# dan-lee-gh/monte-carlo-gp

Hardware: AMD Instinct MI355X
Metric: race-simulations/sec (20 drivers, 60 laps) (higher is better)
Workload: dtype f64

## Files before the change

### monte_carlo_gp_amd/csrc/mcgp_hip.hip

```cpp
#include "../../include/mcgp.h"
#include "params_build.h"
#include "race_kernel.hip.h"
#include "race_kernel_reg.hip.h"
#include "championship.hip.h"
#include "champ_rounds.hip.h"
#include "matchups.hip.h"
#include "resume.hip.h"
#include "trace.hip.h"
#include "strategy.hip.h"
#include "gaps.hip.h"
#include "conditions.hip.h"
#include "stints.hip.h"
#include "moves.hip.h"
#include "fastest.hip.h"
#include "champ_bonus.hip.h"
#include "plan_pack.h"
#include "champ_pack.h"

#define MCGP_FE_FN __host__ __device__ static inline
#include "frontend_exp.h"
#include "elo_update.h"
#include "normal53_table.h"

#include <hip/hip_runtime.h>
// ... 193 lines not shown
    c.d_fe_in = c.d_fe_out = c.d_norm53 = nullptr;
    c.d_fe_pen = nullptr;
    c.work.release();
    if (c.call_start) (void)hipEventDestroy(c.call_start);
    if (c.call_stop) (void)hipEventDestroy(c.call_stop);
    c.call_start = c.call_stop = nullptr;
    for (auto &t : c.timer) {
        if (t.start) (void)hipEventDestroy(t.start);
        if (t.stop) (void)hipEventDestroy(t.stop);
        if (t.d_ticket) (void)hipFree(t.d_ticket);
        t.retire.release();
        t = DeviceCtx::Timer{};
    }
    c.last_timer = -1;
}

size_t lds_limit(size_t device_bytes)
{
    if (const char *e = std::getenv("MCGP_LDS_PER_BLOCK")) {
        const unsigned long long v = std::strtoull(e, nullptr, 10);
        if (v >= 16384 && v < device_bytes) return (size_t)v;
    }
    return device_bytes;
}

int init_ctx_body(int device, DeviceCtx &c)
{
    HIP_TRY(hipSetDevice(device));
    hipDeviceProp_t prop;
    HIP_TRY(hipGetDeviceProperties(&prop, device));
    c.cu_count = prop.multiProcessorCount;
    c.lds_per_block = lds_limit(prop.sharedMemPerBlock);
    for (auto &sl : c.slot) {
        HIP_TRY(hipMalloc(&sl.dev, sizeof(mcgp::KParams)));
        HIP_TRY(hipHostMalloc(&sl.host, sizeof(mcgp::KParams)));
        HIP_TRY(hipEventCreateWithFlags(&sl.uploaded, hipEventDisableTiming));
    }
    HIP_TRY(hipMalloc(&c.d_hist, sizeof(unsigned long long) * MCGP_MAX_CARS * MCGP_MAX_CARS));
    HIP_TRY(hipMalloc(&c.d_grid, MCGP_MAX_CARS));
    HIP_TRY(hipMalloc(&c.d_order1, MCGP_MAX_CARS));
    HIP_TRY(hipMalloc(&c.d_fe_in, sizeof(double) * 4 * MCGP_MAX_CARS));
    HIP_TRY(hipMalloc(&c.d_fe_pen, sizeof(int32_t) * MCGP_MAX_CARS));
    HIP_TRY(hipMalloc(&c.d_fe_out, sizeof(double) * MCGP_MAX_CARS * MCGP_MAX_CARS));
    HIP_TRY(hipMalloc(&c.d_norm53, sizeof(mcgp_normal53_table_bits)));
    HIP_TRY(hipMemcpy(c.d_norm53, mcgp_normal53_table_bits, sizeof(mcgp_normal53_table_bits), hipMemcpyHostToDevice));
    HIP_TRY(hipFuncSetAttribute(reinterpret_cast<const void *>(&mcgp::race_kernel),
                                hipFuncAttributeMaxDynamicSharedMemorySize, (int)c.lds_per_block));
    HIP_TRY(hipFuncSetAttribute(reinterpret_cast<const void *>(&mcgp::race_resume_kernel),
                                hipFuncAttributeMaxDynamicSharedMemorySize, (int)c.lds_per_block));
    HIP_TRY(hipFuncSetAttribute(reinterpret_cast<const void *>(&mcgp::race_trace_kernel),
                                hipFuncAttributeMaxDynamicSharedMemorySize, (int)c.lds_per_block));
    return MCGP_OK;
}

int ensure_ctx_locked(int device, DeviceCtx &c)
{
    if (c.ready) return MCGP_OK;
    const int rc = init_ctx_body(device, c);
    if (rc != MCGP_OK) {
        release_ctx(c);
        return rc;
    }
    c.ready = true;
    return MCGP_OK;
}

int build_params(const mcgp_config *cfg, const mcgp_drivers *drv, const double *grid_probs, uint32_t n,
                 mcgp::KParams *kp)
{
    const char *err = "";
    const int rc = mcgp::build_params(cfg, drv, grid_probs, n, kp, &err);
    return rc == MCGP_OK ? rc : fail(rc, err);
}

using KernelFn = void (*)(const mcgp::KParams *, uint64_t, uint64_t, uint32_t, uint32_t, unsigned long long *,
                          uint8_t *, const uint8_t *, uint32_t, uint32_t *, uint32_t *);

}

namespace mcgp {
#define X(N_)                                                                                                                   \
    extern template __global__ void race_kernel_reg<N_>(const KParams *, uint64_t, uint64_t, uint32_t, uint32_t,               \
                                                        unsigned long long *, uint8_t *, const uint8_t *, uint32_t, uint32_t *, \
                                                        uint32_t *);                                                           \
    extern template __global__ void race_kernel_reg<N_, kSmallBlockWaves>(const KParams *, uint64_t, uint64_t, uint32_t,       \
                                                                          uint32_t, unsigned long long *, uint8_t *,           \
                                                                          const uint8_t *, uint32_t, uint32_t *, uint32_t *);  \
    extern template __global__ void race_kernel_reg_wide<N_>(const KParams *, uint64_t, uint64_t, uint32_t, uint32_t,          \
                                                             unsigned long long *, uint8_t *, const uint8_t *, uint32_t,       \
                                                             uint32_t *, uint32_t *, const double *);                          \
    extern template __global__ void race_kernel_reg_batch<N_>(const KParams *, const BatchItem *, uint32_t, uint64_t,          \
                                                              unsigned long long *, uint32_t, uint32_t *, uint32_t *);
MCGP_REG_SIZES(X)
#undef X
}

namespace {

using BatchKernelFn = void (*)(const mcgp::KParams *, const mcgp::BatchItem *, uint32_t, uint64_t, unsigned long long *,
                               uint32_t, uint32_t *, uint32_t *);
using WideKernelFn = void (*)(const mcgp::KParams *, uint64_t, uint64_t, uint32_t, uint32_t, unsigned long long *,
                              uint8_t *, const uint8_t *, uint32_t, uint32_t *, uint32_t *, const double *);

struct RegKernels {
    KernelFn reg, small;
    WideKernelFn wide;
    BatchKernelFn batch;
};
const RegKernels kRegKernels[] = {
#define X(N_) {&mcgp::race_kernel_reg<N_>, &mcgp::race_kernel_reg<N_, mcgp::kSmallBlockWaves>, \
               &mcgp::race_kernel_reg_wide<N_>, &mcgp::race_kernel_reg_batch<N_>},
    MCGP_REG_SIZES(X)
#undef X
};
static_assert(sizeof(kRegKernels) / sizeof(kRegKernels[0]) == MCGP_MAX_CARS, "one entry per field size 1..32");

const RegKernels *reg_kernels(uint32_t n) { return n >= 1 && n <= MCGP_MAX_CARS ? &kRegKernels[n - 1] : nullptr; }

bool force_generic()
{
    const char *e = std::getenv("MCGP_FORCE_GENERIC");
    return e && e[0] == '1';
}

KernelFn select_kernel(const mcgp::KParams &kp, bool *is_reg)
{
    const RegKernels *rk = reg_kernels((uint32_t)kp.n);
    *is_reg = rk && !force_generic() && mcgp::reg_kernel_serves(kp);
    return *is_reg ? rk->reg : &mcgp::race_kernel;
}

int check_wide(const mcgp::KParams &kp)
{
// ... 173 lines not shown
int launch(DeviceCtx &c, const mcgp::KParams &kp, uint64_t n_sims, uint64_t sim_offset, uint64_t seed,
           hipStream_t stream, unsigned long long *d_hist, uint8_t *d_orders, const uint8_t *d_fixed_grid,
           const FrontEnd &fe = FrontEnd())
{
    if (n_sims == 0) return MCGP_OK;
    bool is_reg = false;
    KernelFn kernel = select_kernel(kp, &is_reg);
    WideKernelFn wide = nullptr;
    if (kp.wide) {
        const int rc = check_wide(kp);
        if (rc != MCGP_OK) return rc;
        wide = reg_kernels((uint32_t)kp.n)->wide;
        HIP_TRY(hipFuncSetAttribute(reinterpret_cast<const void *>(wide), hipFuncAttributeMaxDynamicSharedMemorySize,
                                    (int)c.lds_per_block));
        is_reg = true;
        kernel = nullptr;
    }
    DeviceCtx::Slot *sl = nullptr;
    if (!fe.on)
        for (auto &cand : c.slot)
            if (cand.used && cand.shareable && std::memcmp(cand.host, &kp, sizeof(kp)) == 0) { sl = &cand; break; }
    if (!sl) {
        sl = &c.slot[c.next_slot];
        c.next_slot = (c.next_slot + 1) % kParamSlots;
        if (sl->used)
            for (auto &rd : sl->reader)
                if (rd.live) {
                    HIP_TRY(hipEventSynchronize(rd.done));
                    rd.live = false;
                }
        std::memcpy(sl->host, &kp, sizeof(kp));
        sl->used = true;
        sl->shareable = !fe.on;
        HIP_TRY(hipMemcpyAsync(sl->dev, sl->host, sizeof(kp), hipMemcpyHostToDevice, stream));
        if (fe.on) {
            hipLaunchKernelGGL(grid_probs_kernel, dim3(1), dim3(mcgp::kMaxCars), 0, stream, c.d_fe_in, c.d_fe_pen,
                               (int)kp.n, sl->dev->grid_probs);
            HIP_TRY(hipGetLastError());
        }
        HIP_TRY(hipEventRecord(sl->uploaded, stream));
        sl->upload_stream = stream;
    } else if (sl->upload_stream != stream) {
        HIP_TRY(hipStreamWaitEvent(stream, sl->uploaded, 0));
    }
    int ti = -1;
    {
        const int rc = claim_timer(c, stream, &ti);
        if (rc != MCGP_OK) return rc;
    }
    c.timer[ti].seq = ++c.timer_seq;
    if (!c.timer[ti].d_ticket) return fail(MCGP_E_HIP, "no work counter for this stream");
    HIP_TRY(hipEventRecord(c.timer[ti].start, stream));
    const uint64_t cap = max_sims_per_launch();
    uint32_t grid = 0, block = 0, lds = 0;
    bool small_shape = false;
    auto resource_error = [](hipError_t e) {
        return e == hipErrorOutOfMemory || e == hipErrorInvalidValue || e == hipErrorLaunchOutOfResources ||
               e == hipErrorInvalidConfiguration;
    };
    for (uint64_t done = 0; done < n_sims; done += cap) {
        const uint64_t m = (n_sims - done) < cap ? (n_sims - done) : cap;
        for (;;) {
            const KernelFn k = small_shape ? reg_kernels((uint32_t)kp.n)->small : kernel;
            launch_geometry(c, (uint32_t)kp.n, is_reg, wide ? reinterpret_cast<KernelFn>(wide) : k, m, &grid, &block, &lds,
                            wide ? mcgp::wide_block_waves(kp.n) : small_shape ? mcgp::kSmallBlockWaves : 0, wide != nullptr,
                            kp.total_laps);
            const bool may_shrink = is_reg && !wide && !small_shape;
// ... 356 lines not shown
int32_t mcgp_run_batch(uint32_t n_problems, const mcgp_config *cfgs, const mcgp_drivers *drvs,
                       const double *const *grid_probs, uint32_t n, uint64_t n_sims, const uint64_t *sim_offsets,
                       const uint64_t *seeds, int32_t device, uint64_t *hist_out)
{
    if (!cfgs || !drvs || !grid_probs || !seeds || !hist_out) return fail(MCGP_E_BAD_ARG, "a batch array is NULL");
    if (n_problems < 1 || n_problems > 4096) return fail(MCGP_E_BAD_ARG, "n_problems must be in [1, 4096]");
    if (n_sims >= 0xFFFFFE00ull) return fail(MCGP_E_BAD_ARG, "n_sims per problem must be below 2^32 - 512 in a batch");
    if (n_sims == 0) return MCGP_OK;
    std::vector<mcgp::KParams> kps;
    std::vector<mcgp::BatchItem> items;
    std::vector<uint32_t> shared_index, solo_index;
    std::vector<mcgp::KParams> solo_kps;
    const bool generic = force_generic();
    const RegKernels *rk = reg_kernels(n);
    {
        mcgp::KParams kp;
        for (uint32_t p = 0; p < n_problems; ++p) {
            if (!grid_probs[p]) return fail(MCGP_E_BAD_ARG, "a grid_probs pointer of the batch is NULL");
            int rc = build_params(&cfgs[p], &drvs[p], grid_probs[p], n, &kp);
            if (rc == MCGP_OK) rc = check_wide(kp);
            if (rc != MCGP_OK) return rc;
            if (!rk || generic || kp.wide || !mcgp::reg_kernel_serves(kp)) {
                solo_index.push_back(p);
                solo_kps.push_back(kp);
            } else {
                shared_index.push_back(p);
                kps.push_back(kp);
                items.push_back(mcgp::BatchItem{sim_offsets ? sim_offsets[p] : 0ull, seeds[p]});
            }
        }
    }
    const uint32_t n_shared = (uint32_t)kps.size();
    const size_t cells = (size_t)n * n;
    Counts counts;
    const int rc = on_device(device, true, [&](DeviceCtx &c) -> int {
        const int waves = mcgp::reg_block_waves((int)n);
        const uint32_t block = (uint32_t)waves * 64u;
        const size_t lds = mcgp::shared_lds_bytes_reg((int)n) + (size_t)block * mcgp::per_thread_lds_bytes_reg((int)n) +
                           mcgp::kBatchLdsExtra;
        int reg_cap = 4 * mcgp::reg_min_waves((int)n);
        int blocks_per_cu = (int)(c.lds_per_block / lds);
        if (blocks_per_cu * waves > reg_cap) blocks_per_cu = reg_cap / waves;
        if (blocks_per_cu < 1) blocks_per_cu = 1;
        const uint32_t n_chunks = (uint32_t)((n_sims + 63) / 64);
        const uint64_t n_tasks = ((uint64_t)n_shared * n_chunks + (uint64_t)waves - 1) / (uint64_t)waves;
        uint64_t grid = (uint64_t)c.cu_count * (uint64_t)blocks_per_cu;
        if (grid > n_tasks) grid = n_tasks;
        Layout ws;
        const size_t o_kps = ws.add(sizeof(mcgp::KParams) * n_shared), o_items = ws.add(sizeof(mcgp::BatchItem) * n_shared);
        const size_t o_hist = ws.add(sizeof(unsigned long long) * cells * n_problems);
        const size_t o_ticket = ws.add(sizeof(uint32_t) * n_shared);
        const size_t o_retire = ws.add(mcgp::reg_retire_ws_bytes((int)n, (size_t)grid * block));
        int r = c.work.reserve(ws.bytes);
        if (r != MCGP_OK) return r;
        unsigned long long *d_hist = c.work.at<unsigned long long>(o_hist);
        HIP_TRY(hipMemsetAsync(d_hist, 0, o_retire - o_hist, nullptr));
        if (n_shared) {
            const BatchKernelFn kernel = rk->batch;
            HIP_TRY(hipFuncSetAttribute(reinterpret_cast<const void *>(kernel), hipFuncAttributeMaxDynamicSharedMemorySize,
                                        (int)c.lds_per_block));
            HIP_TRY(hipMemcpyAsync(c.work.at(o_kps), kps.data(), sizeof(mcgp::KParams) * n_shared, hipMemcpyHostToDevice, nullptr));
            HIP_TRY(hipMemcpyAsync(c.work.at(o_items), items.data(), sizeof(mcgp::BatchItem) * n_shared, hipMemcpyHostToDevice,
                                   nullptr));
            hipLaunchKernelGGL(kernel, dim3((uint32_t)grid), dim3(block), lds, nullptr, c.work.at<const mcgp::KParams>(o_kps),
                               c.work.at<const mcgp::BatchItem>(o_items), n_shared, n_sims, d_hist, n_chunks,
                               c.work.at<uint32_t>(o_ticket), c.work.at<uint32_t>(o_retire));
            HIP_TRY(hipGetLastError());
            note_launch(c, (uint32_t)grid, block, (uint32_t)lds, "mcgp::race_kernel_reg_batch<%u>", n);
        }
        for (size_t j = 0; j < solo_index.size(); ++j) {
            const uint32_t p = solo_index[j];
            r = launch(c, solo_kps[j], n_sims, sim_offsets ? sim_offsets[p] : 0ull, seeds[p], nullptr,
                       d_hist + (n_shared + j) * cells, nullptr, nullptr);
            if (r != MCGP_OK) return r;
        }
        return counts.download(d_hist, cells * n_problems);
    });
    if (rc != MCGP_OK) return rc;
    std::vector<Counts::Seg> segs;
    for (uint32_t p : shared_index) segs.push_back({hist_out + (size_t)p * cells, cells});
    for (uint32_t p : solo_index) segs.push_back({hist_out + (size_t)p * cells, cells});
    counts.add_to(segs);
    return MCGP_OK;
}

struct ChampRoundsOut {
    uint64_t *round_hist, *contend, *secure, *team_round_hist, *team_contend, *team_secure;
};

struct ChampBonus {
    const int32_t *points, *within;
    uint64_t *bonus_hist, *fastest_hist;
};

static int32_t run_championship(uint32_t n_races, const mcgp_config *cfgs, const mcgp_drivers *drvs,
                                const double *const *grid_probs, uint32_t n, uint64_t n_sims, uint64_t sim_offset,
                                const uint64_t *seeds, const int32_t *points, const uint8_t *countback,
                                const int32_t *init_points, const int32_t *init_counts, const int32_t *team,
                                uint32_t n_teams, int32_t device, uint64_t *champ_hist, uint64_t *team_hist,
// ... 1047 lines not shown
```

### monte_carlo_gp_amd/csrc/params_build.h

```cpp
#pragma once
#include "../../include/mcgp.h"
#include "normal_table.h"
#include "race_common.hip.h"

#include <cmath>
#include <cstring>

namespace mcgp {

inline uint64_t threshold(double p)
{
    if (!(p > 0.0)) return 0;
    const double x = p * 4294967296.0;
    if (x >= 4294967296.0) return 4294967296ull;
    return (uint64_t)std::ceil(x);
}

inline uint64_t threshold53(double p)
{
    if (!(p > 0.0)) return 0;
    const double x = p * 9007199254740992.0;
    if (x >= 9007199254740992.0) return 9007199254740992ull;
    return (uint64_t)std::ceil(x);
}
// ... 48 lines not shown
        if (cfg->comp_optimal_laps[c] < 0 || cfg->comp_optimal_laps[c] > 50000)
            { *err = "comp_optimal_laps out of range"; return MCGP_E_BAD_ARG; }
    }
    for (uint32_t d = 0; d < n; ++d) {
        const double deg = drv->tire_deg[d];
        kp->base_pace[d] = drv->base_pace[d];
        kp->factor[d] = deg > 0 ? deg / 0.05 : 1.0;
        kp->tire_deg[d] = deg;
        kp->variance[d] = drv->variance[d];
        kp->t_dnf1[d] = threshold(drv->team_dnf[d] * 4.0);
        kp->t_dnf[d] = threshold(drv->lap_dnf[d]);
        kp->t53_dnf1[d] = threshold53(drv->team_dnf[d] * 4.0);
        kp->q64_dnf[d] = survival64(drv->lap_dnf[d]);
        const double pit_deg = drv->tire_deg_pit[d];
        for (int c = 0; c < 5; ++c) {
            int opt = cfg->comp_optimal_laps[c];
            if (pit_deg > 0.05) opt = (int)((double)opt * 0.85);
            else if (pit_deg < 0.02) opt = (int)((double)opt * 1.1);
            kp->opt_laps[d * kCompStride + c] = (uint16_t)opt;
        }
    }
    if (grid_probs)
        for (uint32_t d = 0; d < n; ++d)
            for (uint32_t s = 0; s < n; ++s) {
                const double p = grid_probs[(size_t)d * n + s];
                if (!(p >= 0.0)) { *err = "grid_probs has a negative or NaN entry"; return MCGP_E_BAD_ARG; }
                kp->grid_probs[(size_t)d * n + s] = p;
            }
    static_assert(sizeof(mcgp_normal_table_bits) == sizeof(kp->normal_bits), "normal table size");
    std::memcpy(kp->normal_bits, mcgp_normal_table_bits, sizeof(kp->normal_bits));
    return MCGP_OK;
}

}
```

### monte_carlo_gp_amd/csrc/race_common.hip.h

```cpp
#pragma once
#include <hip/hip_runtime.h>
#include <stdint.h>

namespace mcgp {

constexpr int kMaxCars = 32;
constexpr int kNormalRows = 448;
constexpr int kNormal53Rows = 784;
constexpr int kNormal53RowBytes = 64;
constexpr int kCompStride = 8;

constexpr uint32_t kPurposeGrid = 0u << 16;
constexpr uint32_t kPurposeEvent = 1u << 16;
constexpr uint32_t kPurposeCar = 2u << 16;
constexpr uint32_t kPurposeOvt = 3u << 16;
constexpr uint32_t kPurposeRetire = 4u << 16;

__host__ __device__ inline uint32_t retire_next_threshold(uint32_t S, uint32_t q)
{
    return (uint32_t)(((uint64_t)S * (uint64_t)q) >> 32);
}
__host__ __device__ inline uint32_t draw_retirement_lap(uint32_t w, uint64_t t, int L)
{
    if (t == 0ull) return 0u;
    const uint32_t q = (uint32_t)(4294967296ull - t);
    uint32_t S = q;
    for (int k = 2; k <= L; ++k) {
        if (!(w < S)) return (uint32_t)k;
        S = retire_next_threshold(S, q);
    }
    return 0u;
}
__host__ __device__ inline uint32_t draw_retirement_lap_after(uint32_t w, uint64_t t, int k, int L)
{
    const uint32_t r = draw_retirement_lap(w, t, L - k + 1);
    return r == 0u ? 0u : (uint32_t)(k - 1) + r;
}

struct KParams {
    int32_t n, total_laps, track, pop_sh, pop_mh, pad0;
    double pit_loss, overtake_delta, drs_delta, dirty_thr, dirty_pen;
    double overtake_delta_31;
    uint64_t t_red, t_sc, t_vsc, t_vsc_tire;
    double comp_deg[kCompStride], comp_delta[kCompStride];
    double base_pace[kMaxCars];
    double factor[kMaxCars];
    double tire_deg[kMaxCars];
    double variance[kMaxCars];
    uint64_t t_dnf1[kMaxCars];
    uint64_t t_dnf[kMaxCars];
    uint16_t opt_laps[kMaxCars * kCompStride];
    double grid_probs[kMaxCars * kMaxCars];
    uint32_t normal_bits[kNormalRows * 4];
    int32_t wide, pad1;
    uint64_t t53_red, t53_sc, t53_vsc, t53_vsc_tire;
    uint64_t t53_dnf1[kMaxCars];
    uint64_t q64_dnf[kMaxCars];
};

constexpr size_t kSharedTableBytes =
    kNormalRows * 16
    + 4 * kMaxCars * 8
    + 2 * kMaxCars * 8
    + kMaxCars * kCompStride * 2
    + 2 * kCompStride * 8
    + kMaxCars * kMaxCars * 4;
__host__ __device__ constexpr size_t per_thread_lds_bytes(int n) { return (size_t)n * (8 + 8 + 4 + 1 + 2); }

__device__ __forceinline__ uint32_t xor3_key(uint32_t a, uint32_t b, uint32_t key)
{
#if defined(__HIP_DEVICE_COMPILE__)
    uint32_t r;
    asm("v_bitop3_b32 %0, %1, %2, %3 bitop3:0x96" : "=v"(r) : "v"(a), "v"(b), "s"(key));
    return r;
#else
    return a ^ b ^ key;
#endif
}

__device__ __forceinline__ void philox4x32_10(uint32_t c0, uint32_t c1, uint32_t c2, uint32_t c3,
                                              uint32_t k0, uint32_t k1,
                                              uint32_t &o0, uint32_t &o1, uint32_t &o2, uint32_t &o3)
{
#pragma unroll
    for (int r = 0; r < 10; ++r) {
        const uint64_t p0 = (uint64_t)0xD2511F53u * c0;
        const uint64_t p1 = (uint64_t)0xCD9E8D57u * c2;
        const uint32_t n0 = xor3_key((uint32_t)(p1 >> 32), c1, k0);
        const uint32_t n2 = xor3_key((uint32_t)(p0 >> 32), c3, k1);
        c1 = (uint32_t)p1;
        c3 = (uint32_t)p0;
// ... 93 lines not shown
```

### monte_carlo_gp_amd/csrc/race_isa.hip.h

```cpp
#ifndef MCGP_RACE_ISA_H
#define MCGP_RACE_ISA_H
#include <hip/hip_runtime.h>

namespace mcgp {

__device__ __forceinline__ void minmax_f64(double a, double b, double &lo, double &hi)
{
    asm("v_min_f64 %0, %1, %2" : "=v"(lo) : "v"(a), "v"(b));
    asm("v_max_f64 %0, %1, %2" : "=v"(hi) : "v"(a), "v"(b));
}

__device__ __forceinline__ double max_f64(double a, double b)
{
    double r;
    asm("v_max_f64 %0, %1, %2" : "=v"(r) : "v"(a), "v"(b));
    return r;
}

__device__ __forceinline__ double max_abs_f64(double a, double b)
{
    double r;
    asm("v_max_f64 %0, |%1|, %2" : "=v"(r) : "v"(a), "v"(b));
    return r;
}
// ... 384 lines not shown
{
    const int lo = __builtin_amdgcn_readlane(__double2loint(x), lane);
    const int hi = __builtin_amdgcn_readlane(__double2hiint(x), lane);
    return __hiloint2double(hi, lo);
}
__device__ __forceinline__ double bpermute_f64(double x, int src_lane)
{
    const int lo = __builtin_amdgcn_ds_bpermute(src_lane << 2, __double2loint(x));
    const int hi = __builtin_amdgcn_ds_bpermute(src_lane << 2, __double2hiint(x));
    return __hiloint2double(hi, lo);
}
__device__ __forceinline__ uint32_t next_ticket(uint32_t *counter, uint32_t , uint32_t , int )
{
    uint32_t t = 0u;
    if (__builtin_amdgcn_mbcnt_hi(~0u, __builtin_amdgcn_mbcnt_lo(~0u, 0u)) == 0u)
        t = __hip_atomic_fetch_add(counter, 1u, __ATOMIC_RELAXED, __HIP_MEMORY_SCOPE_AGENT);
    return (uint32_t)__builtin_amdgcn_readfirstlane((int)t);
}
__device__ __forceinline__ uint32_t peek_ticket(const uint32_t *counter)
{
    return __hip_atomic_load(counter, __ATOMIC_RELAXED, __HIP_MEMORY_SCOPE_AGENT);
}
__device__ __forceinline__ uint32_t first_lane_with(bool pred)
{
    const unsigned long long m = __ballot(pred);
    return m ? (uint32_t)__builtin_ctzll(m) : 64u;
}
#define MCGP_ANY(pred) (__any((int)(pred)) != 0)
__device__ __forceinline__ void pin(uint32_t &x) { asm volatile("" : "+v"(x)); }
__device__ __forceinline__ void pin(double &x) { asm volatile("" : "+v"(x)); }
__device__ __forceinline__ void pin_scalar(uint32_t &x) { asm volatile("" : "+s"(x)); }
template <typename T>
__device__ __forceinline__ void pin_ptr(const T *&p) { asm volatile("" : "+s"(p)); }

__device__ __forceinline__ uint32_t lds_base_of(const void *p)
{
    return (uint32_t)(uintptr_t)(const MCGP_LDS void *)p;
}

}
#endif
```

### monte_carlo_gp_amd/csrc/race_kernel_reg.hip.h

```cpp
#pragma once
#include "race_common.hip.h"
#include "race_isa.hip.h"
#include "sort_networks.h"

#include <utility>

#ifndef MCGP_STAT
#define MCGP_STAT(what, value)
#endif
#ifndef MCGP_TRACE_PASS
#define MCGP_TRACE_PASS(sim, lap, pass, n_cand)
#endif
#ifndef MCGP_COOPERATIVE_EVENTS
#define MCGP_COOPERATIVE_EVENTS 1
#endif
#ifndef MCGP_GRID_EXACT
#define MCGP_GRID_EXACT 0
#endif
#ifndef MCGP_WIDE_EXACT
#define MCGP_WIDE_EXACT 0
#endif
#ifndef MCGP_WIDE_TIE_SHIFT
#define MCGP_WIDE_TIE_SHIFT 0
#endif
// ... 538 lines not shown
        philox4x32_10(c0l, c1l, (uint32_t)lap, kPurposeOvt | (uint32_t)(8 * pass + chunk), k0l, k1l, o0, o1, o2, o3);
        lds_st<uint32_t>(w_row_(0), o0);
        lds_st<uint32_t>(w_row_(1), o1);
        lds_st<uint32_t>(w_row_(2), o2);
        lds_st<uint32_t>(w_row_(3), o3);
        philox4x32_10(c0l, c1l, (uint32_t)lap, kPurposeOvt | kCompanion | (uint32_t)(8 * pass + chunk), k0l, k1l, o0, o1, o2, o3);
        lds_st<uint32_t>(w_row_(4), o0);
        lds_st<uint32_t>(w_row_(5), o1);
        lds_st<uint32_t>(w_row_(6), o2);
        lds_st<uint32_t>(w_row_(7), o3);
        uint32_t h = 0u;
#pragma unroll
        for (int i = 1; i < N; ++i) {
            const uint32_t r = (uint32_t)__popc(cur & ((1u << i) - 1u)) * (uint32_t)(B * 4) + tid4;
            const uint64_t u = uniform53(lds_ld<uint32_t>(G::oW + r), lds_ld<uint32_t>(G::oW + (uint32_t)(4 * B * 4) + r));
            h |= u < thr64[i] ? (1u << i) : 0u;
        }
        hits53 |= h & cur;
        rest = m;
    }
    return hits53;
}
template <int N>
struct PkWords {
    uint32_t v[N];
};
template <int N, class G>
__device__ __attribute__((noinline)) uint32_t wide_pass_exact_fn(PkWords<N> field, double od31, uint32_t lap, uint32_t pass, uint32_t c0l,
                                                                 uint32_t c1l, uint32_t k0l_, uint32_t k1l_, uint32_t tid)
{
    return wide_pass_exact_body<N, G>(field.v, od31, lap, pass, c0l, c1l, uniform_u32(k0l_), uniform_u32(k1l_), tid);
}

template <int N, bool WIDE = false, class G = RegGeo<N>>
__device__ __forceinline__ void reg_simulate(const KParams *__restrict__ P, unsigned char *smem, uint32_t tid,
                                             uint32_t *__restrict__ ticket, uint64_t n_sims,
                                             uint64_t sim_offset, uint32_t seed_lo, uint32_t seed_hi,
                                             uint8_t *__restrict__ orders, const uint8_t *__restrict__ fixed_grid,
                                             uint32_t n_chunks, uint32_t *__restrict__ retire_ws_base, uint32_t ws_stride,
                                             uint32_t ws_first_lane, const double *__restrict__ norm53 = nullptr)
{
    constexpr int B = G::B;
    constexpr int kStepBatch = 4;
    constexpr bool kLean = WIDE && wide_min_waves(N) >= 3;
    constexpr int kPaceBatch = 5;
    static_assert(kStepBatch % 4 == 0, "a Philox block serves four consecutive places");
    const uint32_t tid4 = tid * 4u, tid8 = tid * 8u;
    const int L = P->total_laps;
    const int track = P->track;

    uint32_t *s_hist = reinterpret_cast<uint32_t *>(smem + G::oHist);

    auto w_row = [&](int r) -> uint32_t { return G::oW + (uint32_t)r * (B * 4) + tid4; };
    auto l_row = [&](int d) -> uint32_t { return G::oLast + (uint32_t)d * (B * 8) + tid8; };
    auto last_of = [&](uint32_t p) -> uint32_t { return ((p >> k3IdShift) & 31u) * (uint32_t)(B * 8) + tid8; };
    auto grid_byte = [&](int pos) -> uint32_t { return G::oW + (uint32_t)(pos >> 2) * (B * 4) + tid4 + (uint32_t)(pos & 3); };
    auto norm_row = [&](uint32_t off) -> float4 { return lds_ld_float4(G::oNorm - kNormalRowBias * 16u + off); };
    constexpr uint32_t kRareHi = (kNormal53HiBias + (uint32_t)(G::kNorm53First > 16 ? G::kNorm53First : 16)) << 16;
    [[maybe_unused]] auto norm53_row = [&](uint32_t hi, double (&c)[8]) {
        const uint32_t a = (hi >> 16) * (uint32_t)kNorm53LdsStride + (G::oNorm53 - (kNormal53HiBias + (uint32_t)G::kNorm53First) * (uint32_t)kNorm53LdsStride);
#pragma unroll
        for (int k = 0; k < 4; ++k) {
            const f64x2 v = lds_ld_f64x2(a + 16u * k);
            c[2 * k] = v.x;
            c[2 * k + 1] = v.y;
        }
// ... 212 lines not shown
                    if (i + 1 <= 3 && 1.0 < sd) sd = 1.0;
                    cum[i] = 0.0 + (base_lap - sd * 0.5);
                    pk[i] = p + (1u << k3AgeShift);
                }
            }
        }
#pragma unroll 1
        for (int d = 0; d < N; ++d) lds_st<double>(l_row(d), 0.0);
        network_sort<N>(cum, pk);
        update_positions_reg<N>(cum, pk, false, dirty_thr);

        constexpr uint32_t kNoKey = 0x7FFFu;
        auto retirements_after = [&](const uint32_t *ws, uint32_t after) -> uint32_t {
            const uint32_t n_out = ws[(size_t)N * ws_stride];
            uint32_t k1 = kNoKey, k2 = kNoKey, left = 0u;
#pragma unroll 1
            for (uint32_t k = 0; k < n_out; ++k) {
                const uint32_t e = ws[(size_t)k * ws_stride];
                if (e > after) {
                    ++left;
                    const uint32_t hi = e > k1 ? e : k1;
                    k1 = e < k1 ? e : k1;
                    k2 = hi < k2 ? hi : k2;
                }
            }
            return k1 | (k2 << 16) | (left > 2u ? 0x80000000u : 0u);
        };
        uint32_t next_out;
        {
            uint32_t tid_w = tid;
            pin(tid_w);
            uint32_t *retire_ws = retire_ws_base + ws_first_lane + tid_w;
            uint32_t n_out = 0u, k1 = kNoKey, k2 = kNoKey;
#pragma unroll 1
            for (int d0 = 0; d0 < N; d0 += 4) {
                uint32_t rw[4];
                philox4x32_10(c0, c1, 0u, kPurposeRetire | (uint32_t)(d0 >> 2), seed_lo, seed_hi, rw[0], rw[1], rw[2], rw[3]);
                uint32_t survived[4];
                if constexpr (WIDE) {
                    uint32_t rx[4];
                    philox4x32_10(c0, c1, 0u, kPurposeRetire | kCompanion | (uint32_t)(d0 >> 2), seed_lo, seed_hi, rx[0], rx[1], rx[2], rx[3]);
                    uint64_t Q[4], q64[4], S64[4];
#pragma unroll
                    for (int j = 0; j < 4; ++j) {
                        Q[j] = ((uint64_t)rw[j] << 32) | ((uint64_t)(rx[j] >> 11) << 11);
                        q64[j] = d0 + j < N ? P->q64_dnf[d0 + j] : 0ull;
                        S64[j] = q64[j];
                        survived[j] = 0u;
                    }
                    if (G::chain_fits(L)) {
                        uint32_t a = G::oChain + (uint32_t)d0 * 8u;
#pragma unroll 1
                        for (int k = 2; k <= L; ++k) {
#pragma unroll
                            for (int j = 0; j < 4; ++j) survived[j] += Q[j] < lds_ld<uint64_t>(a + 8u * j) ? 1u : 0u;
                            a += G::kChainStride;
                        }
                    } else {
#pragma unroll 1
                    for (int k = 2; k <= L; ++k) {
#pragma unroll
                        for (int j = 0; j < 4; ++j) {
                            survived[j] += Q[j] < S64[j] ? 1u : 0u;
                            S64[j] = __umul64hi(S64[j], q64[j]);
                        }
                    }
                    }
                } else {
                uint32_t q[4], S[4];
#pragma unroll
                for (int j = 0; j < 4; ++j) {
                    const uint64_t t = d0 + j < N ? P->t_dnf[d0 + j] : 0ull;
                    q[j] = (uint32_t)(4294967296ull - t);
                    S[j] = q[j];
                    survived[j] = 0u;
                }
#pragma unroll 1
                for (int k = 2; k <= L; ++k) {
#pragma unroll
                    for (int j = 0; j < 4; ++j) {
                        survived[j] += rw[j] < S[j] ? 1u : 0u;
                        S[j] = retire_next_threshold(S[j], q[j]);
                    }
                }
                }
#pragma unroll
                for (int j = 0; j < 4; ++j) {
                    const int d = d0 + j;
                    if (d >= N) continue;
                    if (P->t_dnf[d] == 0ull) continue;
                    const uint32_t out_lap = 2u + survived[j];
                    if (out_lap <= (uint32_t)L) {
                        const uint32_t key = (out_lap << 5) | (uint32_t)d;
                        if (n_out == 2u) {
                            retire_ws[0] = k1;
                            retire_ws[(size_t)ws_stride] = k2;
                        }
                        if (n_out >= 2u) retire_ws[(size_t)n_out * ws_stride] = key;
                        ++n_out;
                        const uint32_t hi = key > k1 ? key : k1;
                        k1 = key < k1 ? key : k1;
                        k2 = hi < k2 ? hi : k2;
                    }
                }
            }
            if (n_out > 2u) retire_ws[(size_t)N * ws_stride] = n_out;
            next_out = k1 | (k2 << 16) | (n_out > 2u ? 0x80000000u : 0u);
        }

        int drs_disabled_until = 0;
#pragma unroll 1
        for (int lap = 2; lap <= L; ++lap) {
            const int remaining_laps = L - lap;
            uint32_t lane_l = tid;
            pin(lane_l);
            const uint64_t sim_l = sim_offset + ((uint64_t)chunk * 64ull + (uint64_t)(lane_l & 63u));
            uint32_t c0l = (uint32_t)sim_l, c1l = (uint32_t)(sim_l >> 32);
// ... 531 lines not shown
{
    using G = WideGeo<N>;
    extern __shared__ __align__(16) unsigned char smem[];
    if ((int)blockDim.x != G::B || lds_base_of(smem) != 0u) __builtin_trap();
    reg_load_tables<N, G>(P, smem, threadIdx.x, norm53);
    __syncthreads();
    reg_simulate<N, true, G>(P, smem, threadIdx.x, ticket, n_sims, sim_offset, seed_lo, seed_hi, orders, fixed_grid, n_chunks,
                             retire_ws, (uint32_t)(gridDim.x * G::B), (uint32_t)(blockIdx.x * G::B), norm53);
    __syncthreads();
    reg_flush_hist<N, G>(smem, threadIdx.x, hist);
}

struct BatchItem {
    uint64_t sim_offset, seed;
};
template <int N>
__device__ __forceinline__ void batch_problem(const KParams *__restrict__ P, unsigned char *smem, uint32_t *__restrict__ ticket,
                                              uint64_t n_sims, uint64_t sim_offset, uint64_t seed, uint32_t n_chunks,
                                              uint32_t *__restrict__ retire_ws, unsigned long long *__restrict__ hist)
{
    using G = RegGeo<N>;
    reg_load_tables<N>(P, smem, threadIdx.x);
    __syncthreads();
    reg_simulate<N>(P, smem, threadIdx.x, ticket, n_sims, sim_offset, (uint32_t)seed, (uint32_t)(seed >> 32),
                    nullptr, nullptr, n_chunks, retire_ws, (uint32_t)(gridDim.x * G::B), (uint32_t)(blockIdx.x * G::B));
    __syncthreads();
    reg_flush_hist<N>(smem, threadIdx.x, hist);
    __syncthreads();
}
template <int N>
__global__ void __launch_bounds__(RegGeo<N>::B, reg_min_waves(N))
race_kernel_reg_batch(const KParams *__restrict__ P, const BatchItem *__restrict__ items, uint32_t n_problems,
                      uint64_t n_sims, unsigned long long *__restrict__ hist, uint32_t n_chunks,
                      uint32_t *__restrict__ tickets, uint32_t *__restrict__ retire_ws)
{
    using G = RegGeo<N>;
    extern __shared__ __align__(16) unsigned char smem[];
    if ((int)blockDim.x != G::B || lds_base_of(smem) != 0u) __builtin_trap();
    uint32_t p = (uint32_t)(((uint64_t)blockIdx.x * n_problems) / gridDim.x);
    uint32_t visited = 0u;
    for (;;) {
        if (threadIdx.x < 64u) {
            uint32_t found = 0xFFFFFFFFu, seen = visited;
            while (seen < n_problems) {
                const uint32_t k = seen + threadIdx.x;
                uint32_t q = p + (k - visited);
                if (q >= n_problems) q -= n_problems;
                const uint32_t lane = first_lane_with(k < n_problems && peek_ticket(&tickets[q]) < n_chunks);
                if (lane < 64u) {
                    found = seen + lane;
                    break;
                }
                seen += 64u;
            }
            if (threadIdx.x == 0u) lds_st<uint32_t>(G::kBytes, found);
        }
        __syncthreads();
        const uint32_t found = lds_ld<uint32_t>(G::kBytes);
        if (found == 0xFFFFFFFFu) break;
        p += found - visited;
        if (p >= n_problems) p -= n_problems;
        visited = found + 1u;
        const BatchItem it = items[p];
        batch_problem<N>(P + p, smem, tickets + p, n_sims, it.sim_offset, it.seed, n_chunks, retire_ws, hist + (size_t)p * N * N);
        p += 1u;
        if (p >= n_problems) p -= n_problems;
    }
}
constexpr size_t kBatchLdsExtra = 16;

}
```

### monte_carlo_gp_amd/csrc/reg_inst.hip

```cpp
#include "race_kernel_reg.hip.h"

#ifndef MCGP_INST_N
#error "compile with -DMCGP_INST_N=<field size>"
#endif

namespace mcgp {
template __global__ void race_kernel_reg<MCGP_INST_N>(const KParams *, uint64_t, uint64_t, uint32_t, uint32_t,
                                                      unsigned long long *, uint8_t *, const uint8_t *, uint32_t, uint32_t *, uint32_t *);
template __global__ void race_kernel_reg<MCGP_INST_N, kSmallBlockWaves>(const KParams *, uint64_t, uint64_t, uint32_t, uint32_t,
                                                                        unsigned long long *, uint8_t *, const uint8_t *, uint32_t,
                                                                        uint32_t *, uint32_t *);
template __global__ void race_kernel_reg_batch<MCGP_INST_N>(const KParams *, const BatchItem *, uint32_t, uint64_t,
                                                            unsigned long long *, uint32_t, uint32_t *, uint32_t *);
template __global__ void race_kernel_reg_wide<MCGP_INST_N>(const KParams *, uint64_t, uint64_t, uint32_t, uint32_t,
                                                           unsigned long long *, uint8_t *, const uint8_t *, uint32_t, uint32_t *,
                                                           uint32_t *, const double *);
}
```

Before: 152.9 million.

## Precompute per-driver retirement thresholds on host and binary-search them in kernel

Per-driver DNF survival thresholds for every lap are now built on the host and placed behind the KParams block, both in the per-slot upload and in the batch path with a strided layout. The kernel finds each retirement lap with a branchless binary search over that table in global memory, replacing the O(L) loop that recomputed thresholds lap by lap. This cuts retirement-draw ALU work from linear to logarithmic in laps, at the cost of a larger parameter upload, a host-side table build, and dependent global loads during the search.

```diff
diff --git a/monte_carlo_gp_amd/csrc/mcgp_hip.hip b/monte_carlo_gp_amd/csrc/mcgp_hip.hip
--- a/monte_carlo_gp_amd/csrc/mcgp_hip.hip
+++ b/monte_carlo_gp_amd/csrc/mcgp_hip.hip
@@ -249,8 +249,8 @@
     c.cu_count = prop.multiProcessorCount;
     c.lds_per_block = lds_limit(prop.sharedMemPerBlock);
     for (auto &sl : c.slot) {
-        HIP_TRY(hipMalloc(&sl.dev, sizeof(mcgp::KParams)));
-        HIP_TRY(hipHostMalloc(&sl.host, sizeof(mcgp::KParams)));
+        HIP_TRY(hipMalloc(&sl.dev, mcgp::kRetireTabOffset + mcgp::kRetireTabMaxBytes));
+        HIP_TRY(hipHostMalloc(&sl.host, mcgp::kRetireTabOffset + mcgp::kRetireTabMaxBytes));
         HIP_TRY(hipEventCreateWithFlags(&sl.uploaded, hipEventDisableTiming));
     }
     HIP_TRY(hipMalloc(&c.d_hist, sizeof(unsigned long long) * MCGP_MAX_CARS * MCGP_MAX_CARS));
@@ -307,7 +307,8 @@
                                                              unsigned long long *, uint8_t *, const uint8_t *, uint32_t,       \
                                                              uint32_t *, uint32_t *, const double *);                          \
     extern template __global__ void race_kernel_reg_batch<N_>(const KParams *, const BatchItem *, uint32_t, uint64_t,          \
-                                                              unsigned long long *, uint32_t, uint32_t *, uint32_t *);
+                                                              unsigned long long *, uint32_t, uint32_t *, uint32_t *,      \
+                                                              uint32_t);
 MCGP_REG_SIZES(X)
 #undef X
 }
@@ -315,7 +316,7 @@
 namespace {
 
 using BatchKernelFn = void (*)(const mcgp::KParams *, const mcgp::BatchItem *, uint32_t, uint64_t, unsigned long long *,
-                               uint32_t, uint32_t *, uint32_t *);
+                               uint32_t, uint32_t *, uint32_t *, uint32_t);
 using WideKernelFn = void (*)(const mcgp::KParams *, uint64_t, uint64_t, uint32_t, uint32_t, unsigned long long *,
                               uint8_t *, const uint8_t *, uint32_t, uint32_t *, uint32_t *, const double *);
 
@@ -555,7 +556,9 @@
         std::memcpy(sl->host, &kp, sizeof(kp));
         sl->used = true;
         sl->shareable = !fe.on;
-        HIP_TRY(hipMemcpyAsync(sl->dev, sl->host, sizeof(kp), hipMemcpyHostToDevice, stream));
+        mcgp::build_retire_table(kp, kp.wide != 0, reinterpret_cast<unsigned char *>(sl->host) + mcgp::kRetireTabOffset);
+        const size_t upload = mcgp::kRetireTabOffset + mcgp::retire_table_bytes(kp.n, kp.total_laps, kp.wide != 0);
+        HIP_TRY(hipMemcpyAsync(sl->dev, sl->host, upload, hipMemcpyHostToDevice, stream));
         if (fe.on) {
             hipLaunchKernelGGL(grid_probs_kernel, dim3(1), dim3(mcgp::kMaxCars), 0, stream, c.d_fe_in, c.d_fe_pen,
                                (int)kp.n, sl->dev->grid_probs);
@@ -978,6 +981,14 @@
     }
     const uint32_t n_shared = (uint32_t)kps.size();
     const size_t cells = (size_t)n * n;
+    size_t param_stride = 0;
+    for (const mcgp::KParams &k : kps) param_stride = std::max(param_stride, mcgp::retire_table_bytes(k.n, k.total_laps, false));
+    param_stride = mcgp::kRetireTabOffset + (param_stride + 255) / 256 * 256;
+    std::vector<unsigned char> blocks(param_stride * n_shared);
+    for (uint32_t j = 0; j < n_shared; ++j) {
+        std::memcpy(blocks.data() + param_stride * j, &kps[j], sizeof(mcgp::KParams));
+        mcgp::build_retire_table(kps[j], false, blocks.data() + param_stride * j + mcgp::kRetireTabOffset);
+    }
     Counts counts;
     const int rc = on_device(device, true, [&](DeviceCtx &c) -> int {
         const int waves = mcgp::reg_block_waves((int)n);
@@ -993,7 +1004,7 @@
         uint64_t grid = (uint64_t)c.cu_count * (uint64_t)blocks_per_cu;
         if (grid > n_tasks) grid = n_tasks;
         Layout ws;
-        const size_t o_kps = ws.add(sizeof(mcgp::KParams) * n_shared), o_items = ws.add(sizeof(mcgp::BatchItem) * n_shared);
+        const size_t o_kps = ws.add(blocks.size()), o_items = ws.add(sizeof(mcgp::BatchItem) * n_shared);
         const size_t o_hist = ws.add(sizeof(unsigned long long) * cells * n_problems);
         const size_t o_ticket = ws.add(sizeof(uint32_t) * n_shared);
         const size_t o_retire = ws.add(mcgp::reg_retire_ws_bytes((int)n, (size_t)grid * block));
@@ -1005,12 +1016,12 @@
             const BatchKernelFn kernel = rk->batch;
             HIP_TRY(hipFuncSetAttribute(reinterpret_cast<const void *>(kernel), hipFuncAttributeMaxDynamicSharedMemorySize,
                                         (int)c.lds_per_block));
-            HIP_TRY(hipMemcpyAsync(c.work.at(o_kps), kps.data(), sizeof(mcgp::KParams) * n_shared, hipMemcpyHostToDevice, nullptr));
+            HIP_TRY(hipMemcpyAsync(c.work.at(o_kps), blocks.data(), blocks.size(), hipMemcpyHostToDevice, nullptr));
             HIP_TRY(hipMemcpyAsync(c.work.at(o_items), items.data(), sizeof(mcgp::BatchItem) * n_shared, hipMemcpyHostToDevice,
                                    nullptr));
             hipLaunchKernelGGL(kernel, dim3((uint32_t)grid), dim3(block), lds, nullptr, c.work.at<const mcgp::KParams>(o_kps),
                                c.work.at<const mcgp::BatchItem>(o_items), n_shared, n_sims, d_hist, n_chunks,
-                               c.work.at<uint32_t>(o_ticket), c.work.at<uint32_t>(o_retire));
+                               c.work.at<uint32_t>(o_ticket), c.work.at<uint32_t>(o_retire), (uint32_t)param_stride);
             HIP_TRY(hipGetLastError());
             note_launch(c, (uint32_t)grid, block, (uint32_t)lds, "mcgp::race_kernel_reg_batch<%u>", n);
         }
diff --git a/monte_carlo_gp_amd/csrc/params_build.h b/monte_carlo_gp_amd/csrc/params_build.h
--- a/monte_carlo_gp_amd/csrc/params_build.h
+++ b/monte_carlo_gp_amd/csrc/params_build.h
@@ -104,4 +104,33 @@
     return MCGP_OK;
 }
 
+static_assert(MCGP_MAX_LAPS == kMaxLaps && MCGP_MAX_CARS == kMaxCars, "limits of the retirement table");
+
+inline void build_retire_table(const KParams &kp, bool wide, void *out)
+{
+    const int L = kp.total_laps;
+    const size_t row = retire_row_entries(L);
+    std::memset(out, 0, retire_table_bytes(kp.n, L, wide));
+    for (int d = 0; d < kp.n; ++d) {
+        if (kp.t_dnf[d] == 0ull) continue;
+        if (wide) {
+            uint64_t *S = static_cast<uint64_t *>(out) + (size_t)d * row;
+            const uint64_t q = kp.q64_dnf[d];
+            uint64_t s = q;
+            for (int k = 2; k <= L; ++k) {
+                S[k - 2] = s;
+                s = (uint64_t)(((unsigned __int128)s * q) >> 64);
+            }
+        } else {
+            uint32_t *S = static_cast<uint32_t *>(out) + (size_t)d * row;
+            const uint32_t q = (uint32_t)(4294967296ull - kp.t_dnf[d]);
+            uint32_t s = q;
+            for (int k = 2; k <= L; ++k) {
+                S[k - 2] = s;
+                s = retire_next_threshold(s, q);
+            }
+        }
+    }
 }
+
+}
diff --git a/monte_carlo_gp_amd/csrc/race_common.hip.h b/monte_carlo_gp_amd/csrc/race_common.hip.h
--- a/monte_carlo_gp_amd/csrc/race_common.hip.h
+++ b/monte_carlo_gp_amd/csrc/race_common.hip.h
@@ -30,6 +30,24 @@
         S = retire_next_threshold(S, q);
     }
     return 0u;
+}
+__host__ __device__ inline int retire_search_rounds(int L) { return L > 1 ? 32 - __builtin_clz((unsigned)(L - 1)) : 0; }
+__host__ __device__ inline uint32_t retire_row_entries(int L) { return 1u << retire_search_rounds(L); }
+__host__ __device__ constexpr uint32_t retire_table_rows(int n) { return ((uint32_t)n + 3u) & ~3u; }
+template <typename T>
+__host__ __device__ inline uint32_t retire_search_step(T w, const T *row, uint32_t at, uint32_t span)
+{
+    const T S = *reinterpret_cast<const T *>(reinterpret_cast<const unsigned char *>(row) + at + (span - (uint32_t)sizeof(T)));
+    return at + (w < S ? span : 0u);
+}
+template <typename T>
+__host__ __device__ inline uint32_t retirement_lap_from_table(T w, const T *S, int L)
+{
+    uint32_t at = 0u;
+    for (uint32_t span = retire_row_entries(L) * (uint32_t)sizeof(T) >> 1; span >= (uint32_t)sizeof(T); span >>= 1)
+        at = retire_search_step(w, S, at, span);
+    const uint32_t lap = 2u + at / (uint32_t)sizeof(T);
+    return lap <= (uint32_t)L ? lap : 0u;
 }
 __host__ __device__ inline uint32_t draw_retirement_lap_after(uint32_t w, uint64_t t, int k, int L)
 {
@@ -57,6 +75,17 @@
     uint64_t t53_dnf1[kMaxCars];
     uint64_t q64_dnf[kMaxCars];
 };
+constexpr size_t kRetireTabOffset = (sizeof(KParams) + 255) / 256 * 256;
+constexpr int kMaxLaps = 1000;
+constexpr size_t kRetireTabMaxBytes = (size_t)kMaxCars * 1024 * 8;
+__host__ __device__ inline size_t retire_table_bytes(int n, int L, bool wide)
+{
+    return (size_t)retire_table_rows(n) * retire_row_entries(L) * (wide ? 8u : 4u);
+}
+__host__ __device__ inline const void *retire_table_behind(const KParams *P)
+{
+    return reinterpret_cast<const unsigned char *>(P) + kRetireTabOffset;
+}
 
 constexpr size_t kSharedTableBytes =
     kNormalRows * 16
diff --git a/monte_carlo_gp_amd/csrc/race_isa.hip.h b/monte_carlo_gp_amd/csrc/race_isa.hip.h
--- a/monte_carlo_gp_amd/csrc/race_isa.hip.h
+++ b/monte_carlo_gp_amd/csrc/race_isa.hip.h
@@ -440,6 +440,12 @@
 __device__ __forceinline__ void pin_scalar(uint32_t &x) { asm volatile("" : "+s"(x)); }
 template <typename T>
 __device__ __forceinline__ void pin_ptr(const T *&p) { asm volatile("" : "+s"(p)); }
+#define MCGP_GLOBAL __attribute__((address_space(1)))
+template <typename T>
+__device__ __forceinline__ T global_ld(const void *base, uint32_t off)
+{
+    return *(const MCGP_GLOBAL T *)((const MCGP_GLOBAL unsigned char *)base + off);
+}
 
 __device__ __forceinline__ uint32_t lds_base_of(const void *p)
 {
diff --git a/monte_carlo_gp_amd/csrc/race_kernel_reg.hip.h b/monte_carlo_gp_amd/csrc/race_kernel_reg.hip.h
--- a/monte_carlo_gp_amd/csrc/race_kernel_reg.hip.h
+++ b/monte_carlo_gp_amd/csrc/race_kernel_reg.hip.h
@@ -594,6 +594,25 @@
     return wide_pass_exact_body<N, G>(field.v, od31, lap, pass, c0l, c1l, uniform_u32(k0l_), uniform_u32(k1l_), tid);
 }
 
+template <typename T>
+__device__ __forceinline__ void retire_search4(const T (&w)[4], const void *__restrict__ tab, uint32_t first_row,
+                                               uint32_t row_bytes, uint32_t (&survived)[4])
+{
+    const unsigned char *rows = static_cast<const unsigned char *>(tab) + first_row;
+    uint32_t at[4] = {0u, 0u, 0u, 0u};
+#pragma unroll 1
+    for (uint32_t span = row_bytes >> 1; span >= (uint32_t)sizeof(T); span >>= 1) {
+        T S[4];
+#pragma unroll
+        for (int j = 0; j < 4; ++j)
+            S[j] = global_ld<T>(rows + ((uint32_t)j * row_bytes + span - (uint32_t)sizeof(T)), at[j]);
+#pragma unroll
+        for (int j = 0; j < 4; ++j) at[j] += w[j] < S[j] ? span : 0u;
+    }
+#pragma unroll
+    for (int j = 0; j < 4; ++j) survived[j] = at[j] / (uint32_t)sizeof(T);
+}
+
 template <int N, bool WIDE = false, class G = RegGeo<N>>
 __device__ __forceinline__ void reg_simulate(const KParams *__restrict__ P, unsigned char *smem, uint32_t tid,
                                              uint32_t *__restrict__ ticket, uint64_t n_sims,
@@ -872,6 +891,12 @@
             pin(tid_w);
             uint32_t *retire_ws = retire_ws_base + ws_first_lane + tid_w;
             uint32_t n_out = 0u, k1 = kNoKey, k2 = kNoKey;
+            const KParams *Pt = P;
+            pin_ptr(Pt);
+            const void *retire_tab = retire_table_behind(Pt);
+            uint32_t laps_t = (uint32_t)L;
+            pin_scalar(laps_t);
+            const uint32_t row_bytes = retire_row_entries((int)laps_t) * (uint32_t)(WIDE ? 8u : 4u);
 #pragma unroll 1
             for (int d0 = 0; d0 < N; d0 += 4) {
                 uint32_t rw[4];
@@ -880,12 +905,10 @@
                 if constexpr (WIDE) {
                     uint32_t rx[4];
                     philox4x32_10(c0, c1, 0u, kPurposeRetire | kCompanion | (uint32_t)(d0 >> 2), seed_lo, seed_hi, rx[0], rx[1], rx[2], rx[3]);
-                    uint64_t Q[4], q64[4], S64[4];
+                    uint64_t Q[4];
 #pragma unroll
                     for (int j = 0; j < 4; ++j) {
                         Q[j] = ((uint64_t)rw[j] << 32) | ((uint64_t)(rx[j] >> 11) << 11);
-                        q64[j] = d0 + j < N ? P->q64_dnf[d0 + j] : 0ull;
-                        S64[j] = q64[j];
                         survived[j] = 0u;
                     }
                     if (G::chain_fits(L)) {
@@ -897,32 +920,10 @@
                             a += G::kChainStride;
                         }
                     } else {
-#pragma unroll 1
-                    for (int k = 2; k <= L; ++k) {
-#pragma unroll
-                        for (int j = 0; j < 4; ++j) {
-                            survived[j] += Q[j] < S64[j] ? 1u : 0u;
-                            S64[j] = __umul64hi(S64[j], q64[j]);
-                        }
-                    }
+                        retire_search4(Q, retire_tab, (uint32_t)d0 * row_bytes, row_bytes, survived);
                     }
                 } else {
-                uint32_t q[4], S[4];
-#pragma unroll
-                for (int j = 0; j < 4; ++j) {
-                    const uint64_t t = d0 + j < N ? P->t_dnf[d0 + j] : 0ull;
-                    q[j] = (uint32_t)(4294967296ull - t);
-                    S[j] = q[j];
-                    survived[j] = 0u;
-                }
-#pragma unroll 1
-                for (int k = 2; k <= L; ++k) {
-#pragma unroll
-                    for (int j = 0; j < 4; ++j) {
-                        survived[j] += rw[j] < S[j] ? 1u : 0u;
-                        S[j] = retire_next_threshold(S[j], q[j]);
-                    }
-                }
+                    retire_search4(rw, retire_tab, (uint32_t)d0 * row_bytes, row_bytes, survived);
                 }
 #pragma unroll
                 for (int j = 0; j < 4; ++j) {
@@ -1520,7 +1521,7 @@
 __global__ void __launch_bounds__(RegGeo<N>::B, reg_min_waves(N))
 race_kernel_reg_batch(const KParams *__restrict__ P, const BatchItem *__restrict__ items, uint32_t n_problems,
                       uint64_t n_sims, unsigned long long *__restrict__ hist, uint32_t n_chunks,
-                      uint32_t *__restrict__ tickets, uint32_t *__restrict__ retire_ws)
+                      uint32_t *__restrict__ tickets, uint32_t *__restrict__ retire_ws, uint32_t param_stride)
 {
     using G = RegGeo<N>;
     extern __shared__ __align__(16) unsigned char smem[];
@@ -1550,7 +1551,8 @@
         if (p >= n_problems) p -= n_problems;
         visited = found + 1u;
         const BatchItem it = items[p];
-        batch_problem<N>(P + p, smem, tickets + p, n_sims, it.sim_offset, it.seed, n_chunks, retire_ws, hist + (size_t)p * N * N);
+        const KParams *Pp = reinterpret_cast<const KParams *>(reinterpret_cast<const unsigned char *>(P) + (size_t)p * param_stride);
+        batch_problem<N>(Pp, smem, tickets + p, n_sims, it.sim_offset, it.seed, n_chunks, retire_ws, hist + (size_t)p * N * N);
         p += 1u;
         if (p >= n_problems) p -= n_problems;
     }
diff --git a/monte_carlo_gp_amd/csrc/reg_inst.hip b/monte_carlo_gp_amd/csrc/reg_inst.hip
--- a/monte_carlo_gp_amd/csrc/reg_inst.hip
+++ b/monte_carlo_gp_amd/csrc/reg_inst.hip
@@ -11,7 +11,7 @@
                                                                         unsigned long long *, uint8_t *, const uint8_t *, uint32_t,
                                                                         uint32_t *, uint32_t *);
 template __global__ void race_kernel_reg_batch<MCGP_INST_N>(const KParams *, const BatchItem *, uint32_t, uint64_t,
-                                                            unsigned long long *, uint32_t, uint32_t *, uint32_t *);
+                                                            unsigned long long *, uint32_t, uint32_t *, uint32_t *, uint32_t);
 template __global__ void race_kernel_reg_wide<MCGP_INST_N>(const KParams *, uint64_t, uint64_t, uint32_t, uint32_t,
                                                            unsigned long long *, uint8_t *, const uint8_t *, uint32_t, uint32_t *,
                                                            uint32_t *, const double *);
```

After: 154.6 million (median of 6 runs). 1.1% higher.
